# Cogito2012/OpenTAL

Hardware: AMD Instinct MI355X
Metric: clips/sec training step, 256-frame THUMOS14 clips (higher is better)
Workload: dtype bf16

## Files before the change

### opental_amd/csrc/conv1a_wgrad.inc

```
struct W1aArgs {
    ConvArgs c;
    int nblocks, bps;
};

template <bool DYH>
__global__ __launch_bounds__(256, 2) void conv1a_wgrad_direct_kernel(const W1aArgs d) {
    constexpr int PITCH = C1_PITCH;
    constexpr int PATCH = 2 * C1_NR * PITCH;
    constexpr int AP = 192 * 2 + 16;
    __shared__ __attribute__((aligned(16))) unsigned char lds[PATCH + 64 * AP];
    unsigned char* const patch = lds;
    unsigned char* const dyT = lds + PATCH;
    const ConvArgs& a = d.c;
    const ConvGeom& g = a.g;
    const int tid = threadIdx.x, lane = tid & 63;
    const int wave = __builtin_amdgcn_readfirstlane(tid >> 6);
    const TileId tile = xcd_tile(false);
    const int dt = tile.x, split = tile.y;
    const int blk_begin = split * d.bps, blk_end = min(d.nblocks, blk_begin + d.bps);
    const int tiles_h = g.Ho / 2, tiles_t = g.To / 2;
    const int HWo = g.Ho * g.Wo;
    const auto rx = __builtin_amdgcn_make_buffer_rsrc(const_cast<float*>(a.x), 0, (int)a.src_bytes, 0x00020000);
    const auto rdy = __builtin_amdgcn_make_buffer_rsrc(const_cast<float*>(a.dy), 0, (int)a.dy_bytes, 0x00020000);

    for (int i = tid; i < PATCH / 16; i += 256) reinterpret_cast<uint4*>(patch)[i] = make_uint4(0u, 0u, 0u, 0u);

    constexpr int X_ITEMS = 2 * C1_NR * 24, X_ITERS = (X_ITEMS + 255) / 256;
    int xrel[X_ITERS], xlds[X_ITERS], xpr[X_ITERS];
#pragma unroll
    for (int i = 0; i < X_ITERS; ++i) {
        const int item = tid + 256 * i;
        const int pl = item / (C1_NR * 24), rem = item - pl * (C1_NR * 24), rr = rem / 24, q = rem - rr * 24;
        xrel[i] = ((2 * pl) * g.Hi + rr) * g.Wi + 4 * q;
        xlds[i] = item < X_ITEMS ? (pl * C1_NR + rr) * PITCH + (4 * q + 2) * 8 : -1;
        xpr[i] = (pl << 8) | rr;
    }
    constexpr int A_ITERS = DYH ? 64 * 24 / 256 : 64 * 48 / 256;
    unsigned avo[A_ITERS];
    int alds[A_ITERS];
#pragma unroll
    for (int j = 0; j < A_ITERS; ++j) {
        const int item = tid + 256 * j;
        if constexpr (DYH) {
            const int co = item / 24, rem = item - co * 24, run = rem / 6, o = rem - run * 6;
            avo[j] = co < a.M ? (unsigned)(((int64_t)co * g.y_cs + (run >> 1) * HWo + (run & 1) * g.Wo + 8 * o) * 2) : 0xffffffffu;
            alds[j] = co * AP + (run * 48 + 8 * o) * 2;
        } else {
            const int co = item / 48, rem = item - co * 48, run = rem / 12, q = rem - run * 12;
            avo[j] = co < a.M ? (unsigned)(((int64_t)co * g.y_cs + (run >> 1) * HWo + (run & 1) * g.Wo + 4 * q) * 4) : 0xffffffffu;
            alds[j] = co * AP + (run * 48 + 4 * q) * 2;
        }
    }
    const int grp = wave & 1, khalf = wave >> 1;
    const int dh0 = 4 * grp;
    const int lanex = (2 * (8 * (lane >> 5) + ((lane & 15) >> 2)) + 4 * ((lane >> 4) & 1) + (lane & 3)) * 8;
    const unsigned char* const arow = dyT + (lane & 31) * AP + (lane >> 5) * 16;
    typedef __attribute__((address_space(3))) unsigned char lds_byte;
    lds_byte* const xl = (lds_byte*)patch + lanex + dh0 * PITCH;

    int xoffs[6], aoffs[6];
#pragma unroll
    for (int s2 = 0; s2 < 6; ++s2) {
        const int s = 2 * s2 + khalf;
        const int run = s / 3, w16 = s - run * 3, tl = run >> 1, hl = run & 1;
        xoffs[s2] = __builtin_amdgcn_readfirstlane((tl * C1_NR + 2 * hl) * PITCH + (2 * 16 * w16) * 8);
        aoffs[s2] = __builtin_amdgcn_readfirstlane(s * 32);
    }
    f32x16 acc[2][4];
#pragma unroll
    for (int i = 0; i < 2; ++i)
#pragma unroll
        for (int j = 0; j < 4; ++j)
#pragma unroll
            for (int r = 0; r < 16; ++r) acc[i][j][r] = 0.f;

    float4 xv[X_ITERS][3];
    Words4 ra[A_ITERS];
    auto load = [&](int blk) {
        int bid = blk;
        const int th = bid % tiles_h; bid /= tiles_h;
        const int tt0 = bid % tiles_t;
        const int b = bid / tiles_t;
        const int to0 = tt0 * 2, ho0 = th * 2;
        const int ti0 = 2 * to0 - g.pt + dt, hi0 = 2 * ho0 - g.ph;
        const int64_t xb0 = (int64_t)b * g.x_bs + ((int64_t)ti0 * g.Hi + hi0) * g.Wi;
#pragma unroll
        for (int i = 0; i < X_ITERS; ++i) {
            const int pl = xpr[i] >> 8, rr = xpr[i] & 255;
            const bool ok = xlds[i] >= 0 && (unsigned)(ti0 + 2 * pl) < (unsigned)g.Ti && (unsigned)(hi0 + rr) < (unsigned)g.Hi;
            const unsigned vo = ok ? (unsigned)((xb0 + xrel[i]) * 4) : 0xffffffffu;
#pragma unroll
            for (int ci = 0; ci < 3; ++ci) {
                const Words4 v = __builtin_bit_cast(Words4, __builtin_amdgcn_raw_buffer_load_b128(rx, vo, (int)(ci * g.x_cs * 4), 0));
                xv[i][ci] = make_float4(__uint_as_float(v.a), __uint_as_float(v.b), __uint_as_float(v.c), __uint_as_float(v.d));
            }
        }
        const int ybase = (int)(((int64_t)b * g.y_bs + (int64_t)to0 * HWo + ho0 * g.Wo) * (DYH ? 2 : 4));
#pragma unroll
        for (int j = 0; j < A_ITERS; ++j)
            ra[j] = __builtin_bit_cast(Words4, __builtin_amdgcn_raw_buffer_load_b128(rdy, avo[j], ybase, 0));
    };
    if (blk_begin < blk_end) load(blk_begin);
    for (int blk = blk_begin; blk < blk_end; ++blk) {
        __syncthreads();
#pragma unroll
        for (int i = 0; i < X_ITERS; ++i) {
            if (xlds[i] < 0) continue;
            uint2* dst = reinterpret_cast<uint2*>(patch + xlds[i]);
            dst[0] = make_uint2(cvt_pk_bf16(xv[i][0].x, xv[i][1].x), cvt_pk_bf16(xv[i][2].x, 0.f));
            dst[1] = make_uint2(cvt_pk_bf16(xv[i][0].y, xv[i][1].y), cvt_pk_bf16(xv[i][2].y, 0.f));
            dst[2] = make_uint2(cvt_pk_bf16(xv[i][0].z, xv[i][1].z), cvt_pk_bf16(xv[i][2].z, 0.f));
            dst[3] = make_uint2(cvt_pk_bf16(xv[i][0].w, xv[i][1].w), cvt_pk_bf16(xv[i][2].w, 0.f));
        }
#pragma unroll
        for (int j = 0; j < A_ITERS; ++j) {
            if constexpr (DYH) {
                *reinterpret_cast<Words4*>(dyT + alds[j]) = ra[j];
            } else {
                Words2 pk;
                pk.a = cvt_pk_bf16(__builtin_bit_cast(float, ra[j].a), __builtin_bit_cast(float, ra[j].b));
                pk.b = cvt_pk_bf16(__builtin_bit_cast(float, ra[j].c), __builtin_bit_cast(float, ra[j].d));
                *reinterpret_cast<Words2*>(dyT + alds[j]) = pk;
            }
        }
        __syncthreads();
        if (blk + 1 < blk_end) load(blk + 1);
#pragma unroll
        for (int s2 = 0; s2 < 6; ++s2) {
            const bf16x8 av0 = *reinterpret_cast<const bf16x8*>(arow + aoffs[s2]);
            const bf16x8 av1 = *reinterpret_cast<const bf16x8*>(arow + 32 * AP + aoffs[s2]);
#pragma unroll
            for (int j = 0; j < 4; ++j) {
                if (j == 3 && grp) continue;
                const v4s16 lo = __builtin_amdgcn_ds_read_tr16_b64_v4i16(
                    (__attribute__((address_space(3))) v4s16*)(xl + xoffs[s2] + j * PITCH));
                const v4s16 hi = __builtin_amdgcn_ds_read_tr16_b64_v4i16(
                    (__attribute__((address_space(3))) v4s16*)(xl + xoffs[s2] + j * PITCH + 64));
                const bf16x8 bv = {lo[0], lo[1], lo[2], lo[3], hi[0], hi[1], hi[2], hi[3]};
                acc[0][j] = __builtin_amdgcn_mfma_f32_32x32x16_bf16(av0, bv, acc[0][j], 0, 0, 0);
                acc[1][j] = __builtin_amdgcn_mfma_f32_32x32x16_bf16(av1, bv, acc[1][j], 0, 0, 0);
            }
        }
    }

    float* const xch = reinterpret_cast<float*>(lds);
#pragma unroll
    for (int mt = 0; mt < 2; ++mt) {
        __syncthreads();
        if (khalf) {
#pragma unroll
            for (int j = 0; j < 4; ++j)
#pragma unroll
                for (int r = 0; r < 16; ++r) xch[((grp * 4 + j) * 16 + r) * 64 + lane] = acc[mt][j][r];
        }
        __syncthreads();
        if (!khalf) {
#pragma unroll
            for (int j = 0; j < 4; ++j)
#pragma unroll
                for (int r = 0; r < 16; ++r) acc[mt][j][r] += xch[((grp * 4 + j) * 16 + r) * 64 + lane];
        }
    }
    if (khalf) return;

    const bool slabs = a.splits > 1;
    const auto ro = __builtin_amdgcn_make_buffer_rsrc(slabs ? a.slab : a.out, 0, (int)(slabs ? a.slab_bytes : a.out_bytes), 0x00020000);
    const bool accum = !slabs && (a.flags & EPI_ACCUM);
    const int nn = lane & 31, dw = nn >> 2, ci = nn & 3;
#pragma unroll
    for (int j = 0; j < 4; ++j) {
        if (j == 3 && grp) continue;
        const int dh = dh0 + j;
        const unsigned col = (unsigned)(ci * 343 + dt * 49 + dh * 7 + dw);
        const bool okn = ci < 3 && dw < 7;
#pragma unroll
        for (int mt = 0; mt < 2; ++mt)
#pragma unroll
            for (int r = 0; r < 16; ++r) {
                const int m = mt * 32 + (r & 3) + 8 * (r >> 2) + 4 * (lane >> 5);
                const unsigned vo = (okn && m < a.M) ? (((unsigned)(slabs ? split : 0) * (unsigned)a.M + (unsigned)m) * (unsigned)a.N + col) * 4u : 0xffffffffu;
                float v = acc[mt][j][r];
                if (accum) v += __uint_as_float(__builtin_amdgcn_raw_buffer_load_b32(ro, vo, 0, 0));
                __builtin_amdgcn_raw_buffer_store_b32(__float_as_uint(v), ro, vo, 0, 0);
            }
    }
}

int launch_conv1a_wgrad(ConvArgs& a, void* ws, size_t ws_bytes, hipStream_t st) {
    const ConvGeom& g = a.g;
    W1aArgs d;
    d.nblocks = g.B * (g.To / 2) * (g.Ho / 2);
    int splits = OTAL_OPT("OTAL_W1A_SPLITS") > 0 ? OTAL_OPT("OTAL_W1A_SPLITS") : 73;
    if (splits > d.nblocks) splits = d.nblocks;
    const size_t slab1 = (size_t)a.M * a.N * sizeof(float);
    if (splits > 1 && (!ws || ws_bytes < (size_t)splits * slab1)) {
        splits = ws ? (int)(ws_bytes / slab1) : 1;
        if (splits < 2) splits = 1;
    }
    d.bps = (d.nblocks + splits - 1) / splits;
    splits = (d.nblocks + d.bps - 1) / d.bps;
    a.splits = splits;
    a.k_per_split = d.bps;
    a.slab = splits > 1 ? (float*)ws : nullptr;
    a.src_bytes = (unsigned)gather_extent_bytes(g, MODE_FWD);
    a.dy_bytes = (unsigned)(gather_extent_bytes(g, MODE_DGRAD) >> (a.half ? 1 : 0));
    a.flags &= ~EPI_NPAD8;
    set_epilogue_extents<MODE_WGRAD>(a);
    if ((splits > 1 ? a.slab_bytes : a.out_bytes) == 0u) return OTAL_E_UNSUPPORTED;
    d.c = a;
    if (a.half) hipLaunchKernelGGL(conv1a_wgrad_direct_kernel<true>, dim3(7, splits), dim3(256), 0, st, d);
    else hipLaunchKernelGGL(conv1a_wgrad_direct_kernel<false>, dim3(7, splits), dim3(256), 0, st, d);
    if (int e = otal_launch_status()) return e;
    if (splits > 1) return launch_splitk_reduce<MODE_WGRAD>(a, st);
    return 0;
}
```

### opental_amd/csrc/conv_select.h

```cpp
#pragma once
#include <stddef.h>
#include <stdint.h>
#include "conv_index.h"
#include "options.h"

namespace {

enum { MODE_FWD = 0, MODE_DGRAD = 1, MODE_WGRAD = 2 };

constexpr int C1_TT = 2, C1_TR = 2, C1_WO = 48;
constexpr int C1T_TT = 4, C1T_TR = 4;
constexpr int W1_TC = 128;
constexpr int PJ_HW = 36;
constexpr int PW_KS = 32;
constexpr size_t TAB_PAD = 64;
constexpr int CHUNK_PAD = 16;
constexpr int PTAB_PAD = 64;

static inline size_t align256(size_t v) { return (v + 255) & ~(size_t)255; }
static inline size_t tab_bytes(int K) { return (((size_t)K + TAB_PAD) * (2 * sizeof(int)) + 255) & ~(size_t)255; }
static inline int chunk_kp(int K) { return (K + 31) / 32 * 32; }
static inline size_t chunk_tab_bytes(int K) { return align256(((size_t)chunk_kp(K) / 8 + CHUNK_PAD) * (2 * sizeof(int))); }
static inline size_t chunk_wp_bytes(int M, int BM, int K) {
    return align256(((size_t)((M + BM - 1) / BM * BM) * chunk_kp(K) + 64) * sizeof(unsigned short));
}
static inline size_t ptab_bytes(const ConvGeom& g, int cw) {
    return align256(((size_t)g.B * conv_out_positions(g) / cw + PTAB_PAD) * (2 * sizeof(int)));
}
static inline int64_t gather_extent_bytes(const ConvGeom& g, int mode, int esz = 4) {
    if (mode == MODE_FWD) return esz * ((int64_t)(g.B - 1) * g.x_bs + (int64_t)(g.Cin - 1) * g.x_cs + conv_in_positions(g));
    return esz * ((int64_t)(g.B - 1) * g.y_bs + (int64_t)(g.Cout - 1) * g.y_cs + conv_out_positions(g));
}

static inline int choose_bm(int M, bool tall = false) {
    if (tall && M % 192 == 0) return 192;
    const int cand[4] = {128, 96, 64, 32};
    const double pen[4] = {1.00, 1.03, 1.10, 1.30};
    int best = 128;
    double bc = 1e30;
    for (int i = 0; i < 4; ++i) {
        const double c = (double)((M + cand[i] - 1) / cand[i] * cand[i]) * pen[i];
        if (c < bc) { bc = c; best = cand[i]; }
    }
    return best;
}

static inline int choose_splits(int tiles, int K, int prec = 1, bool wgrad = false) {
    const bool wv = wgrad && prec;
    const int target = wv ? 2048 : 512;
    const int minsteps = wv ? 16 : (prec ? 8 : 4);
    const int cap = wv ? 1024 : 384;
    if (tiles >= target * 3 / 4) return 1;
    int want = (target + tiles - 1) / tiles;
    int maxs = K / (minsteps * 32);
    if (maxs < 1) maxs = 1;
    int s = want < maxs ? want : maxs;
    return s < 1 ? 1 : (s > cap ? cap : s);
}

static inline bool conv1a_half_out_ok(const ConvGeom& g, const void* y) {
    return g.y_bs % 8 == 0 && g.y_cs % 8 == 0 && (reinterpret_cast<uintptr_t>(y) & 15) == 0;
}
static inline bool conv1a_direct_eligible(const ConvGeom& g, int mode, int prec, const void* x) {
    if (!prec || mode != MODE_FWD || g.nlev > 1 || OTAL_OPT("OTAL_CONV_NO1A")) return false;
    if (g.Cin != 3 || g.kt != 7 || g.kh != 7 || g.kw != 7 || g.st != 2 || g.sh != 2 || g.sw != 2) return false;
    if (g.pt != 2 || g.ph != 2 || g.pw != 2 || g.Wi != 96 || g.Wo != C1_WO || g.Hi != 2 * g.Ho || g.Ti != 2 * g.To) return false;
    if (g.To % C1_TT || g.Ho % C1_TR || g.x_bs % 4 || g.x_cs % 4 || (reinterpret_cast<uintptr_t>(x) & 15)) return false;
    return (int64_t)g.B * g.To * g.Ho * g.Wo < (1LL << 31);
}
static inline int conv1a_tile_eligible(int To, int Ho) {
    return To % C1T_TT == 0 && Ho % C1T_TR == 0 && !OTAL_OPT("OTAL_CONV_1A_NOTILE");
}
static inline bool conv1a_wgrad_eligible(const ConvGeom& g, int prec, const void* x, const void* dy) {
    if (!prec || g.nlev > 1 || OTAL_OPT("OTAL_CONV_NO1AW")) return false;
    if (g.Cin != 3 || g.Cout > 64 || g.kt != 7 || g.kh != 7 || g.kw != 7 || g.st != 2 || g.sh != 2 || g.sw != 2) return false;
    if (g.pt != 2 || g.ph != 2 || g.pw != 2 || g.Wi != 96 || g.Wo != C1_WO || g.Hi != 2 * g.Ho || g.Ti != 2 * g.To) return false;
    if (g.To % 2 || g.Ho % 2 || g.x_bs % 4 || g.x_cs % 4 || g.y_bs % 4 || g.y_cs % 4) return false;
    if ((reinterpret_cast<uintptr_t>(x) & 15) || (reinterpret_cast<uintptr_t>(dy) & 15)) return false;
    const int64_t ex = gather_extent_bytes(g, MODE_FWD), ey = gather_extent_bytes(g, MODE_DGRAD);
    return ex > 0 && ey > 0 && ex < (1LL << 31) && ey < (1LL << 31);
}

static inline bool proj_fwd_eligible(const ConvGeom& g, int mode, int prec, const void* x, const void* w) {
    if (!prec || mode != MODE_FWD || g.nlev > 1 || OTAL_OPT("OTAL_CONV_NOPROJ")) return false;
    if (g.kt != 1 || g.st != 1 || g.kh != g.Hi || g.kw != g.Wi || g.Ho != 1 || g.Wo != 1 || g.To != g.Ti) return false;
    if (g.Hi * g.Wi != PJ_HW || g.ph != 0 || g.pw != 0 || g.pt != 0 || g.Cin % 4) return false;
    if (((uintptr_t)x & 3) || ((uintptr_t)w & 3)) return false;
    const int64_t ex = gather_extent_bytes(g, MODE_FWD), ew = 4 * (int64_t)g.Cout * g.Cin * PJ_HW;
    return ex > 0 && ex < (1LL << 31) && ew < (1LL << 31);
}
static inline bool proj_wgrad_eligible(const ConvGeom& g, int prec, const void* x, const void* dy) {
    if (!prec || g.nlev > 1 || OTAL_OPT("OTAL_CONV_NOPROJW")) return false;
    if (g.kt != 1 || g.st != 1 || g.kh != g.Hi || g.kw != g.Wi || g.Ho != 1 || g.Wo != 1 || g.To != g.Ti) return false;
    if (g.ph != 0 || g.pw != 0 || g.pt != 0 || g.Hi * g.Wi < 2) return false;
    if (g.To % PW_KS || g.y_cs < g.To || (g.y_cs & 3) || (g.y_bs & 3)) return false;
    if (((uintptr_t)x & 15) || ((uintptr_t)dy & 15) || (g.x_bs & 3) || (g.x_cs & 3)) return false;
    const int64_t ex = gather_extent_bytes(g, MODE_FWD), ey = gather_extent_bytes(g, MODE_DGRAD);
    const int64_t eo = 4 * (int64_t)g.Cout * g.Cin * g.Hi * g.Wi;
    return ex > 0 && ey > 0 && ex < (1LL << 31) && ey < (1LL << 31) && eo < (1LL << 31);
}

static inline bool conv1d_tile_eligible(const ConvGeom& g, int mode, int prec, const void* src, bool emask) {
    if (!prec || mode == MODE_WGRAD || OTAL_OPT("OTAL_CONV_NO1DTILE")) return false;
    if (g.Hi != 1 || g.Wi != 1 || g.Ho != 1 || g.Wo != 1 || g.kh != 1 || g.kw != 1 || g.st != 1 || g.To != g.Ti) return false;
    if (!((g.kt == 1 && g.pt == 0) || (g.kt == 3 && g.pt == 1))) return false;
    if (g.Ti > 4096) return false;
    if ((mode == MODE_FWD ? g.Cout : g.Cin) > 2048) return false;
    const int C = mode == MODE_FWD ? g.Cin : g.Cout;
    if (C % 128) return false;
    if (mode == MODE_DGRAD && emask) return false;
    if (((uintptr_t)src & 3)) return false;
    const int64_t ext = gather_extent_bytes(g, mode);
    return ext > 0 && ext < (1LL << 31);
}
static inline int wgrad1d_chunks(const ConvGeom& g) { return (g.Ti + W1_TC - 1) / W1_TC; }
static inline bool wgrad1d_eligible(const ConvGeom& g, int prec, const void* x, const void* dy) {
    if (!prec || OTAL_OPT("OTAL_CONV_NOW1D")) return false;
    if (g.Hi != 1 || g.Wi != 1 || g.Ho != 1 || g.Wo != 1 || g.kh != 1 || g.kw != 1 || g.st != 1 || g.To != g.Ti) return false;
    if (!((g.kt == 1 && g.pt == 0) || (g.kt == 3 && g.pt == 1))) return false;
    if (g.Cin % 64 || (g.x_bs | g.x_cs | g.y_bs | g.y_cs) & 1) return false;
    if ((reinterpret_cast<uintptr_t>(x) | reinterpret_cast<uintptr_t>(dy)) & 7) return false;
    return (int64_t)g.B * wgrad1d_chunks(g) <= 1024;
}

static inline bool chunk_eligible(const ConvGeom& g, int mode, int prec) {
    if (!prec || mode == MODE_WGRAD) return false;
    const int C = mode == MODE_FWD ? g.Cin : g.Cout;
    if (C % 8 && !(mode == MODE_FWD && g.kw >= 3)) return false;
    const int64_t ext = gather_extent_bytes(g, mode);
    return ext > 0 && ext < (int64_t)0xfffffff0u;
}
static inline bool conv1x1_stream_eligible(const ConvGeom& g, int mode) {
    if (OTAL_OPT("OTAL_CONV_NO1X1STREAM")) return false;
    if (g.kt != 1 || g.kh != 1 || g.kw != 1 || g.st != 1 || g.sh != 1 || g.sw != 1 || g.nlev > 1) return false;
    const int64_t P = conv_out_positions(g);
    if (P != conv_in_positions(g) || P % 128) return false;
    const int C = mode == MODE_FWD ? g.Cin : g.Cout;
    return C % 8 == 0;
}

static inline int direct_bm(const ConvGeom& g, int M) {
    if (M % 96 == 0) return 96;
    if (M > 96) {
        const int64_t nt = (int64_t)g.B * conv_out_positions(g) / 256;
        const int64_t w64 = (M + 63) / 64 * nt, w96 = (M + 95) / 96 * nt;
        if (w64 <= 512 && (w96 + 255) / 256 * 96 < (w64 + 255) / 256 * 64) return 96;
    }
    if (M % 64 == 0) return 64;
    if (M <= 32) return 32;
    const int pad64 = (M + 63) / 64 * 64;
    return (pad64 - M) * 100 <= M * 34 ? 64 : 0;
}
static inline int direct_bnp(const ConvGeom& g, int M) {
    const int BM = direct_bm(g, M);
    if (!BM) return 0;
    const int64_t tm = (M + BM - 1) / BM, NP = (int64_t)g.B * conv_out_positions(g);
    const int min_tiles = OTAL_OPT("OTAL_CONV_DIRECT_MINTILES");
    if (BM == 96 && conv_out_positions(g) % 512 == 0 && tm * (NP / 512) >= OTAL_OPT("OTAL_CONV_DIRECT_MINTILES512")) return 512;
    if (tm * (NP / 256) >= min_tiles) return 256;
    if (tm * (NP / 128) >= min_tiles) return 128;
    return 0;
}
static inline bool direct_eligible(const ConvGeom& g, int mode, int prec, int M) {
    if (OTAL_OPT("OTAL_CONV_NODIRECT") || !prec || mode == MODE_WGRAD || g.nlev > 1) return false;
    if (g.kt != 3 || g.kh != 3 || g.kw != 3 || g.st != 1 || g.sh != 1 || g.sw != 1 || g.pt != 1 || g.ph != 1 || g.pw != 1) return false;
    if (g.To != g.Ti || g.Ho != g.Hi || g.Wo != g.Wi || g.Wi > 24) return false;
    const int P = conv_out_positions(g);
    const int C = mode == MODE_FWD ? g.Cin : g.Cout;
    if (P % 256 || C % 16 || !direct_bnp(g, M)) return false;
    const int64_t ext = gather_extent_bytes(g, mode);
    return ext > 0 && ext < (1LL << 31);
}
static inline size_t direct_wp_bytes(const ConvGeom& g, int M, int C) {
    const int BM = direct_bm(g, M);
    return align256((size_t)((M + BM - 1) / BM * BM) * C * 27 * 2 + 1024);
}

static inline bool wgrad_direct_eligible(const ConvGeom& g, int prec, const void* x, const void* dy) {
    if (!prec || OTAL_OPT("OTAL_CONV_NOWDIRECT") || g.nlev > 1) return false;
    if (g.kt != 3 || g.kh != 3 || g.kw != 3 || g.st != 1 || g.sh != 1 || g.sw != 1 || g.pt != 1 || g.ph != 1 || g.pw != 1) return false;
    if (g.To != g.Ti || g.Ho != g.Hi || g.Wo != g.Wi) return false;
    const bool planes6 = g.Wi == 6 && g.Hi == 6 && g.Ti % 4 == 0;
    const bool planes3 = g.Wi == 3 && g.Hi == 3 && g.Ti % 16 == 0;
    if (!((g.Wi == 24 && g.Hi % 4 == 0) || (g.Wi == 12 && g.Hi == 12) || planes6 || planes3) || g.Cin % 2) return false;
    if (g.Cin < (planes3 ? 32 : 64) || g.Cout < 64) return false;
    if (((uintptr_t)x & 15) || ((uintptr_t)dy & 15) || g.x_cs % 4 || g.x_bs % 4 || g.y_cs % 4 || g.y_bs % 4) return false;
    const int64_t ex = gather_extent_bytes(g, MODE_FWD), ey = gather_extent_bytes(g, MODE_DGRAD);
    return ex > 0 && ey > 0 && ex < (1LL << 31) && ey < (1LL << 31);
}
static inline bool wgrad1x1_wide_eligible(const ConvGeom& g, int prec, const void* x, const void* dy) {
    if (!prec || g.nlev > 1 || OTAL_OPT("OTAL_CONV_NOW1X1")) return false;
    if (g.kt != 1 || g.kh != 1 || g.kw != 1 || g.st != 1 || g.sh != 1 || g.sw != 1) return false;
    if (g.To != g.Ti || g.Ho != g.Hi || g.Wo != g.Wi) return false;
    if (g.Hi == 1 && g.Wi == 1) return false;
    if (conv_out_positions(g) % 32 || (int64_t)g.Cout * g.Cin > (1 << 20)) return false;
    if (((uintptr_t)x & 3) || ((uintptr_t)dy & 3)) return false;
    const int64_t ex = gather_extent_bytes(g, MODE_FWD), ey = gather_extent_bytes(g, MODE_DGRAD);
    return ex > 0 && ey > 0 && ex < (1LL << 31) && ey < (1LL << 31);
}
static inline bool wgrad_pair_mode(const ConvGeom& g, int prec) {
    if (!prec || g.nlev > 1) return false;
    if (g.sw != 2 || g.st > 2 || g.sh > 2 || g.kw > 7 || g.pw > 3 || g.Wo % 8 || conv_out_positions(g) % 32) return false;
    if (g.Wi - (2 * (g.Wo - 8) - g.pw + 6) < 12) return false;
    const int64_t ex = 4 * ((int64_t)(g.B - 1) * g.x_bs + (int64_t)(g.Cin - 1) * g.x_cs + conv_in_positions(g));
    const int64_t ey = 4 * ((int64_t)(g.B - 1) * g.y_bs + (int64_t)(g.Cout - 1) * g.y_cs + conv_out_positions(g));
    return ex > 0 && ey > 0 && ex < (int64_t)0xffffff00u && ey < (int64_t)0xfffffff0u;
}
static inline int wgrad_vector_width(const ConvGeom& g, int prec) {
    if (!prec) return 0;
    if (g.st != 1 || g.sh != 1 || g.sw != 1 || g.nlev > 1) return 0;
    if (g.To != g.Ti || g.Ho != g.Hi || g.Wo != g.Wi) return 0;
    if ((g.kw != 1 && g.kw != 3) || g.pw != (g.kw - 1) / 2) return 0;
    if (conv_out_positions(g) % 32) return 0;
    const int64_t ex = 4 * ((int64_t)(g.B - 1) * g.x_bs + (int64_t)(g.Cin - 1) * g.x_cs + conv_in_positions(g));
    const int64_t ey = 4 * ((int64_t)(g.B - 1) * g.y_bs + (int64_t)(g.Cout - 1) * g.y_cs + conv_out_positions(g));
    if (ex <= 0 || ey <= 0 || ex >= (int64_t)0xfffffff0u || ey >= (int64_t)0xfffffff0u) return 0;
    if (g.kt == 1 && g.kh == 1 && g.kw == 1) return 8;
    if (g.Wi % 8 == 0) return 8;
    if (g.Wi % 4 == 0) return 4;
    if (g.Wi % 2 == 0) return 2;
    return 0;
}

enum ConvKernel {
    CK_GENERIC,
    CK_PROJ, CK_CONV1A, CK_CONV1D_TILE, CK_DIRECT, CK_CHUNKED,
    CK_CONV1A_WGRAD, CK_PROJ_WGRAD, CK_WGRAD_DIRECT, CK_WGRAD1X1, CK_WGRAD_VECTOR, CK_WGRAD1D,
};
static inline const char* conv_kernel_name(int kernel) {
    switch (kernel) {
        case CK_GENERIC: return "generic";
        case CK_PROJ: return "proj";
        case CK_CONV1A: return "conv1a";
        case CK_CONV1D_TILE: return "conv1d_tile";
        case CK_DIRECT: return "direct";
        case CK_CHUNKED: return "chunked";
        case CK_CONV1A_WGRAD: return "conv1a_wgrad";
        case CK_PROJ_WGRAD: return "proj_wgrad";
        case CK_WGRAD_DIRECT: return "wgrad_direct";
        case CK_WGRAD1X1: return "wgrad1x1_wide";
        case CK_WGRAD_VECTOR: return "vector";
        case CK_WGRAD1D: return "wgrad1d";
    }
    return "?";
}
enum ConvPrologue { PRO_NONE = 0, PRO_CHUNK = 1, PRO_PTAB = 2, PRO_DIRECT = 3 };

struct ConvQuery {
    ConvGeom g;
    int mode;
    int precision;
    int accumulate;
    int has_mask;
    uintptr_t x, w, dy, out, mask;
};
struct ConvStep {
    int kernel;
    int cw;
    bool next;
};
struct ConvPlan {
    int n;
    ConvStep step[8];
    int prologue;
};

static inline int conv_step_prologue(int kernel) {
    switch (kernel) {
        case CK_CONV1D_TILE: case CK_CHUNKED: return PRO_CHUNK;
        case CK_DIRECT: return PRO_DIRECT;
        case CK_WGRAD_VECTOR: return PRO_PTAB;
        default: return PRO_NONE;
    }
}

static inline int conv_prologue_layout(const ConvGeom& g, int mode, int prec) {
    if (mode == MODE_WGRAD) return wgrad_pair_mode(g, prec) || wgrad_vector_width(g, prec) ? PRO_PTAB : PRO_NONE;
    if (proj_fwd_eligible(g, mode, prec, nullptr, nullptr)) return PRO_NONE;
    if (conv1a_direct_eligible(g, mode, prec, nullptr)) return PRO_NONE;
    if (direct_eligible(g, mode, prec, mode == MODE_FWD ? g.Cout : g.Cin)) return PRO_DIRECT;
    return chunk_eligible(g, mode, prec) ? PRO_CHUNK : PRO_NONE;
}
static inline size_t conv_prologue_bytes(const ConvGeom& g, int mode, int prec) {
    const int layout = conv_prologue_layout(g, mode, prec);
    const int M = mode == MODE_FWD ? g.Cout : g.Cin;
    if (layout == PRO_CHUNK) {
        const bool kwv = mode == MODE_FWD && (g.Cin % 8) != 0;
        const int K = mode == MODE_FWD ? (kwv ? g.Cin * g.kt * g.kh * 8 : g.Cin * conv_kvol(g)) : g.Cout * conv_kvol(g);
        return chunk_tab_bytes(K) + chunk_wp_bytes(M, choose_bm(M, !kwv), K);
    }
    if (layout == PRO_PTAB) return ptab_bytes(g, g.sw == 2 ? 8 : wgrad_vector_width(g, prec));
    if (layout == PRO_DIRECT) return direct_wp_bytes(g, M, mode == MODE_FWD ? g.Cin : g.Cout);
    return 0;
}

static inline void conv_plan_half(const ConvQuery& q, ConvPlan& p) {
    const ConvGeom& g = q.g;
    const void* px = (const void*)(q.mode == MODE_DGRAD ? q.out : q.x);
    const void* py = (const void*)(q.mode == MODE_FWD ? q.out : q.dy);
    auto add = [&p](int kernel, bool next, int cw = 0) { p.step[p.n++] = ConvStep{kernel, cw, next}; };
    if (!(q.precision & 1) || !(q.precision & 4) || q.accumulate) return;
    if (((uintptr_t)px | (uintptr_t)py) & 15) return;
    if (q.mode == MODE_DGRAD && q.has_mask && (!(q.precision & 16) || (q.mask & 15))) return;
    if (g.nlev > 1) return;
    if (conv_out_positions(g) % 8 || conv_in_positions(g) % 8 || g.x_bs % 8 || g.x_cs % 8 || g.y_bs % 8 || g.y_cs % 8) return;
    if (q.mode == MODE_FWD || q.mode == MODE_DGRAD) {
        const int M = q.mode == MODE_FWD ? g.Cout : g.Cin, C = q.mode == MODE_FWD ? g.Cin : g.Cout;
        if (direct_eligible(g, q.mode, 1, M) && !(g.Wi & 1)) add(CK_DIRECT, false);
        else if (chunk_eligible(g, q.mode, 1) && C % 8 == 0 && conv_in_positions(g) == conv_out_positions(g)) add(CK_CHUNKED, false);
        return;
    }
    const int cw = wgrad_vector_width(g, 1);
    if (wgrad_direct_eligible(g, 1, px, py)) add(CK_WGRAD_DIRECT, true);
    else if (wgrad1x1_wide_eligible(g, 1, px, py)) add(CK_WGRAD1X1, true);
    if (cw) add(CK_WGRAD_VECTOR, false, cw);
}

static inline ConvPlan conv_plan(const ConvQuery& q) {
    ConvPlan p = {};
    const ConvGeom& g = q.g;
    const int prec = q.precision & 1, half = (q.precision >> 2) & 1;
    p.prologue = conv_prologue_layout(g, q.mode, prec);
    if (q.precision & 8) { conv_plan_half(q, p); return p; }
    const void *x = (const void*)q.x, *w = (const void*)q.w, *dy = (const void*)q.dy, *out = (const void*)q.out;
    auto add = [&p](int kernel, bool next, int cw = 0) { p.step[p.n++] = ConvStep{kernel, cw, next}; };
    if (q.mode == MODE_WGRAD) {
        if (conv1a_wgrad_eligible(g, prec, x, dy) && (!half || g.y_bs % 8 + g.y_cs % 8 == 0)) add(CK_CONV1A_WGRAD, !half);
        if (half) return p;
        if (proj_wgrad_eligible(g, prec, x, dy)) add(CK_PROJ_WGRAD, true);
        if (wgrad_direct_eligible(g, prec, x, dy)) add(CK_WGRAD_DIRECT, true);
        if (wgrad1x1_wide_eligible(g, prec, x, dy)) add(CK_WGRAD1X1, true);
        if (wgrad_pair_mode(g, prec)) { add(CK_WGRAD_VECTOR, false, 8); return p; }
        if (const int cw = wgrad_vector_width(g, prec)) { add(CK_WGRAD_VECTOR, false, cw); return p; }
        if (wgrad1d_eligible(g, prec, x, dy)) add(CK_WGRAD1D, true);
        add(CK_GENERIC, false);
        return p;
    }
    const int M = q.mode == MODE_FWD ? g.Cout : g.Cin;
    if (q.mode == MODE_FWD) {
        if (proj_fwd_eligible(g, q.mode, prec, x, w)) add(CK_PROJ, true);
        if (half) {
            if (conv1a_direct_eligible(g, q.mode, prec, x) && conv1a_half_out_ok(g, out)) add(CK_CONV1A, false);
            else if (direct_eligible(g, q.mode, prec, M) && conv1a_half_out_ok(g, out)) add(CK_DIRECT, false);
            return p;
        }
        if (conv1a_direct_eligible(g, q.mode, prec, x)) { add(CK_CONV1A, false); return p; }
    }
    if (half) return p;
    if (conv1d_tile_eligible(g, q.mode, prec, q.mode == MODE_FWD ? x : dy, q.has_mask)) add(CK_CONV1D_TILE, true);
    if (direct_eligible(g, q.mode, prec, M)) add(CK_DIRECT, false);
    else if (chunk_eligible(g, q.mode, prec)) add(CK_CHUNKED, false);
    else add(CK_GENERIC, false);
    return p;
}

static inline int conv_half_storage(const ConvGeom& g, int mode, int precision) {
    if (!(precision & 1) || g.y_bs % 8 || g.y_cs % 8) return 0;
    ConvQuery q = {};
    q.g = g;
    q.mode = mode;
    q.precision = precision | 4;
    const ConvPlan p = conv_plan(q);
    for (int i = 0; i < p.n; ++i)
        if (p.step[i].kernel != CK_PROJ) return 1;
    return 0;
}

}
```

### opental_amd/csrc/options.h

```cpp
#pragma once

struct OtalOption { const char* name; int dflt; };
constexpr OtalOption OTAL_OPTIONS[] = {
    {"OTAL_CONV_1A_NOTILE", 0},           {"OTAL_CONV_1A_WGS", 0},
    {"OTAL_CONV_DIRECT_MINTILES", 140},   {"OTAL_CONV_DIRECT_MINTILES512", 512},
    {"OTAL_CONV_DIRECT_XPF2", 3},         {"OTAL_CONV_NO1A", 0},
    {"OTAL_CONV_NO1AW", 0},               {"OTAL_CONV_NO1DTILE", 0},
    {"OTAL_CONV_NO1X1STREAM", 0},         {"OTAL_CONV_NODIRECT", 0},
    {"OTAL_CONV_NOPROJ", 0},              {"OTAL_CONV_NOPROJW", 0},
    {"OTAL_CONV_NOW1D", 0},               {"OTAL_CONV_NOW1X1", 0},
    {"OTAL_CONV_NOWDIRECT", 0},           {"OTAL_LOSS_NOSTAGE", 0},
    {"OTAL_POOL_NO133", 0},               {"OTAL_POOL_NOROWS", 0},
    {"OTAL_W1A_SPLITS", 0},               {"OTAL_WDIRECT_BLOCKS", 0},
};
constexpr int OTAL_NUM_OPTIONS = sizeof(OTAL_OPTIONS) / sizeof(OTAL_OPTIONS[0]);
constexpr bool otal_streq(const char* a, const char* b) { return *a == *b && (*a == 0 || otal_streq(a + 1, b + 1)); }
constexpr int otal_option_index(const char* name, int i = 0) {
    return i == OTAL_NUM_OPTIONS ? -1 : otal_streq(OTAL_OPTIONS[i].name, name) ? i : otal_option_index(name, i + 1);
}
int* otal_option_slot(int index);
#define OTAL_OPT(name) ([]() -> int {                                                                              \
    constexpr int index_ = otal_option_index(name);                                                              \
    static_assert(index_ >= 0, "unknown option " name " (options.h: OTAL_OPTIONS)");                               \
    static int* const slot_ = otal_option_slot(index_);                                                          \
    return *slot_;                                                                                               \
}())
```

Baseline: 1011.

## Add 4x4-block conv1a weight-gradient kernel with pipelined dy ring and LDS patch reuse

```diff
diff --git a/opental_amd/csrc/conv1a_wgrad.inc b/opental_amd/csrc/conv1a_wgrad.inc
--- a/opental_amd/csrc/conv1a_wgrad.inc
+++ b/opental_amd/csrc/conv1a_wgrad.inc
@@ -186,10 +186,13 @@
     }
 }
 
+#include "conv1a_wgrad_blocks.inc"
+
 int launch_conv1a_wgrad(ConvArgs& a, void* ws, size_t ws_bytes, hipStream_t st) {
     const ConvGeom& g = a.g;
     W1aArgs d;
-    d.nblocks = g.B * (g.To / 2) * (g.Ho / 2);
+    const bool blocks4 = conv1a_wgrad_blocks_eligible(g.To, g.Ho);
+    d.nblocks = blocks4 ? g.B * (g.To / 4) * (g.Ho / 4) : g.B * (g.To / 2) * (g.Ho / 2);
     int splits = OTAL_OPT("OTAL_W1A_SPLITS") > 0 ? OTAL_OPT("OTAL_W1A_SPLITS") : 73;
     if (splits > d.nblocks) splits = d.nblocks;
     const size_t slab1 = (size_t)a.M * a.N * sizeof(float);
@@ -208,7 +211,10 @@
     set_epilogue_extents<MODE_WGRAD>(a);
     if ((splits > 1 ? a.slab_bytes : a.out_bytes) == 0u) return OTAL_E_UNSUPPORTED;
     d.c = a;
-    if (a.half) hipLaunchKernelGGL(conv1a_wgrad_direct_kernel<true>, dim3(7, splits), dim3(256), 0, st, d);
+    if (blocks4) {
+        if (a.half) hipLaunchKernelGGL(conv1a_wgrad_blocks_kernel<true>, dim3(7, splits), dim3(256), 0, st, d);
+        else hipLaunchKernelGGL(conv1a_wgrad_blocks_kernel<false>, dim3(7, splits), dim3(256), 0, st, d);
+    } else if (a.half) hipLaunchKernelGGL(conv1a_wgrad_direct_kernel<true>, dim3(7, splits), dim3(256), 0, st, d);
     else hipLaunchKernelGGL(conv1a_wgrad_direct_kernel<false>, dim3(7, splits), dim3(256), 0, st, d);
     if (int e = otal_launch_status()) return e;
     if (splits > 1) return launch_splitk_reduce<MODE_WGRAD>(a, st);
diff --git a/opental_amd/csrc/conv1a_wgrad_blocks.inc b/opental_amd/csrc/conv1a_wgrad_blocks.inc
--- /dev/null
+++ b/opental_amd/csrc/conv1a_wgrad_blocks.inc
@@ -0,0 +1,212 @@
+constexpr int W1B_NPL = 4, W1B_NR = 13;
+
+template <bool DYH>
+__global__ __launch_bounds__(256, 2) void conv1a_wgrad_blocks_kernel(const W1aArgs d) {
+    constexpr int PITCH = C1_PITCH;
+    constexpr int PLANE = W1B_NR * PITCH;
+    constexpr int HALF = 2 * PLANE;
+    constexpr int PATCH = W1B_NPL * PLANE;
+    constexpr int ESZ = DYH ? 2 : 4;
+    constexpr int G = DYH ? 4 : 2;
+    constexpr int NA = DYH ? 1 : 2;
+    constexpr int STEPS = 12;
+    constexpr int NG = 2 * STEPS / G;
+    constexpr int NS = 3;
+    static_assert(STEPS % G == 0 && 4 % G == 0 && NG % NS == 0, "the ring's slots are compile-time indices");
+    __shared__ __attribute__((aligned(16))) unsigned char lds[PATCH];
+    const ConvArgs& a = d.c;
+    const ConvGeom& g = a.g;
+    const int tid = threadIdx.x, lane = tid & 63;
+    const int wave = __builtin_amdgcn_readfirstlane(tid >> 6);
+    const TileId tile = xcd_tile(false);
+    const int dt = tile.x, split = tile.y;
+    const int blk_begin = split * d.bps, blk_end = min(d.nblocks, blk_begin + d.bps);
+    const int tiles_h = g.Ho / 4, tiles_t = g.To / 4;
+    const int HWo = g.Ho * g.Wo;
+    const auto rx = __builtin_amdgcn_make_buffer_rsrc(const_cast<float*>(a.x), 0, (int)a.src_bytes, 0x00020000);
+    const auto rdy = __builtin_amdgcn_make_buffer_rsrc(const_cast<float*>(a.dy), 0, (int)a.dy_bytes, 0x00020000);
+
+    for (int i = tid; i < PATCH / 16; i += 256) reinterpret_cast<uint4*>(lds)[i] = make_uint4(0u, 0u, 0u, 0u);
+    __syncthreads();
+
+    constexpr int X_ITEMS = 2 * W1B_NR * 24, X_ITERS = (X_ITEMS + 255) / 256;
+    int xitem[X_ITERS];
+#pragma unroll
+    for (int i = 0; i < X_ITERS; ++i) {
+        const int item = tid + 256 * i;
+        const int pl = item / (W1B_NR * 24), rem = item - pl * (W1B_NR * 24), rr = rem / 24, q = rem - rr * 24;
+        xitem[i] = item < X_ITEMS ? (pl | rr << 4 | q << 8) : -1;
+    }
+    const int mt = wave & 1, khalf = wave >> 1;
+    const int lanex = (2 * (8 * (lane >> 5) + ((lane & 15) >> 2)) + 4 * ((lane >> 4) & 1) + (lane & 3)) * 8;
+    typedef __attribute__((address_space(3))) unsigned char lds_byte;
+    lds_byte* const xl = (lds_byte*)lds + lanex + khalf * PLANE;
+    const int co = mt * 32 + (lane & 31);
+    const unsigned avo = co < a.M ? (unsigned)(((int64_t)co * g.y_cs + 8 * (lane >> 5)) * ESZ) : 0xffffffffu;
+
+    f32x16 acc[7];
+#pragma unroll
+    for (int j = 0; j < 7; ++j)
+#pragma unroll
+        for (int r = 0; r < 16; ++r) acc[j][r] = 0.f;
+
+    auto decode = [&](int blk, int& b, int& tt0, int& th) {
+        int bid = blk;
+        th = bid % tiles_h; bid /= tiles_h;
+        tt0 = bid % tiles_t;
+        b = bid / tiles_t;
+    };
+    auto ybase_of = [&](int blk) {
+        int b, tt0, th;
+        decode(blk, b, tt0, th);
+        return (int)(((int64_t)b * g.y_bs + (int64_t)(4 * tt0 + khalf) * HWo + 4 * th * g.Wo) * ESZ);
+    };
+    const int yhalf = 2 * HWo * ESZ;
+    float4 xs[2][3];
+    Words4 ra[NS][G * NA];
+    auto load_xi = [&](int set, int blk, int p, int i) {
+        int b, tt0, th;
+        decode(blk, b, tt0, th);
+        const int ti0 = 2 * (4 * tt0 + 2 * p) - g.pt + dt, hi0 = 2 * (4 * th) - g.ph;
+        const int64_t xb0 = (int64_t)b * g.x_bs + ((int64_t)ti0 * g.Hi + hi0) * g.Wi;
+        int it = xitem[i];
+        asm volatile("" : "+v"(it));
+        const int pl = it & 15, rr = (it >> 4) & 15, q = (it >> 8) & 31;
+        const bool ok = it >= 0 && (unsigned)(ti0 + 2 * pl) < (unsigned)g.Ti && (unsigned)(hi0 + rr) < (unsigned)g.Hi;
+        const unsigned vo = ok ? (unsigned)((xb0 + ((2 * pl) * g.Hi + rr) * g.Wi + 4 * q) * 4) : 0xffffffffu;
+#pragma unroll
+        for (int ci = 0; ci < 3; ++ci) {
+            const Words4 v = __builtin_bit_cast(Words4, __builtin_amdgcn_raw_buffer_load_b128(rx, vo, (int)(ci * g.x_cs * 4), 0));
+            xs[set][ci] = make_float4(__uint_as_float(v.a), __uint_as_float(v.b), __uint_as_float(v.c), __uint_as_float(v.d));
+        }
+    };
+    auto store_xi = [&](int set, int p, int i) {
+        int it = xitem[i];
+        asm volatile("" : "+v"(it));
+        if (it < 0) return;
+        uint2* dst = reinterpret_cast<uint2*>(lds + p * HALF + (it & 15) * PLANE + ((it >> 4) & 15) * PITCH + ((it >> 8) & 31) * 32 + 16);
+        const float4 c0 = xs[set][0], c1 = xs[set][1], c2 = xs[set][2];
+        dst[0] = make_uint2(cvt_pk_bf16(c0.x, c1.x), cvt_pk_bf16(c2.x, 0.f));
+        dst[1] = make_uint2(cvt_pk_bf16(c0.y, c1.y), cvt_pk_bf16(c2.y, 0.f));
+        dst[2] = make_uint2(cvt_pk_bf16(c0.z, c1.z), cvt_pk_bf16(c2.z, 0.f));
+        dst[3] = make_uint2(cvt_pk_bf16(c0.w, c1.w), cvt_pk_bf16(c2.w, 0.f));
+    };
+    auto load_granule = [&](int gi, int yb) {
+        const int j0 = gi * G;
+        const int so = yb + (j0 / STEPS) * yhalf + 16 * (j0 % STEPS) * ESZ;
+#pragma unroll
+        for (int i = 0; i < G * NA; ++i)
+            ra[gi % NS][i] = __builtin_bit_cast(Words4, __builtin_amdgcn_raw_buffer_load_b128(rdy, avo, so + (i / NA) * 16 * ESZ + (i % NA) * 16, 0));
+    };
+    auto frag_a = [&](int j) {
+        const int slot = (j / G) % NS, i = j % G;
+        if constexpr (DYH) {
+            return __builtin_bit_cast(bf16x8, ra[slot][i]);
+        } else {
+            const Words4 lo = ra[slot][2 * i], hi = ra[slot][2 * i + 1];
+            Words4 pk;
+            pk.a = cvt_pk_bf16(__builtin_bit_cast(float, lo.a), __builtin_bit_cast(float, lo.b));
+            pk.b = cvt_pk_bf16(__builtin_bit_cast(float, lo.c), __builtin_bit_cast(float, lo.d));
+            pk.c = cvt_pk_bf16(__builtin_bit_cast(float, hi.a), __builtin_bit_cast(float, hi.b));
+            pk.d = cvt_pk_bf16(__builtin_bit_cast(float, hi.c), __builtin_bit_cast(float, hi.d));
+            return __builtin_bit_cast(bf16x8, pk);
+        }
+    };
+
+    bf16x8 bv[7];
+    int yb_cur = 0;
+    if (blk_begin < blk_end) {
+        yb_cur = ybase_of(blk_begin);
+#pragma unroll
+        for (int gi = 0; gi < NS; ++gi) load_granule(gi, yb_cur);
+        load_xi(0, blk_begin, 0, 0);
+        load_xi(1, blk_begin, 0, 1);
+        store_xi(0, 0, 0);
+        load_xi(0, blk_begin, 0, 2);
+        store_xi(1, 0, 1);
+        store_xi(0, 0, 2);
+        load_xi(0, blk_begin, 1, 0);
+        load_xi(1, blk_begin, 1, 1);
+    }
+    for (int blk = blk_begin; blk < blk_end; ++blk) {
+        const bool more = blk + 1 < blk_end;
+        const int yb_next = more ? ybase_of(blk + 1) : yb_cur;
+#pragma unroll
+        for (int q = 0; q < 6; ++q) {
+            const int p = q / 3;
+            lds_byte* const xh = xl + p * HALF;
+            auto read_b = [&](int jj, int r) {
+                const int xoff = (2 * (jj / 3) + r) * PITCH + (2 * 16 * (jj % 3)) * 8;
+                const v4s16 lo = __builtin_amdgcn_ds_read_tr16_b64_v4i16((__attribute__((address_space(3))) v4s16*)(xh + xoff));
+                const v4s16 hi = __builtin_amdgcn_ds_read_tr16_b64_v4i16((__attribute__((address_space(3))) v4s16*)(xh + xoff + 64));
+                return bf16x8{lo[0], lo[1], lo[2], lo[3], hi[0], hi[1], hi[2], hi[3]};
+            };
+            if (q % 3 == 0) __syncthreads();
+            if (q < 3) store_xi(q & 1, 1, q);
+            else if (more) store_xi(q & 1, 0, q - 3);
+            if (q == 0) load_xi(q & 1, blk, 1, 2);
+            else if (more) {
+                if (q < 4) load_xi(q & 1, blk + 1, 0, q - 1);
+                else load_xi(q & 1, blk + 1, 1, q - 4);
+            }
+            if (q % 3 == 0) {
+#pragma unroll
+                for (int r = 0; r < 7; ++r) bv[r] = read_b(0, r);
+            }
+#pragma unroll
+            for (int s4 = 0; s4 < 4; ++s4) {
+                const int jj = (q % 3) * 4 + s4, j = p * STEPS + jj;
+                const bf16x8 av = frag_a(j);
+                if (j % G == G - 1) {
+                    const int gi = j / G + NS;
+                    if (gi < NG) load_granule(gi, yb_cur);
+                    else load_granule(gi - NG, yb_next);
+                }
+#pragma unroll
+                for (int r = 0; r < 7; ++r) {
+                    acc[r] = __builtin_amdgcn_mfma_f32_32x32x16_bf16(av, bv[r], acc[r], 0, 0, 0);
+                    if (jj + 1 < STEPS) bv[r] = read_b(jj + 1, r);
+                }
+            }
+        }
+        yb_cur = yb_next;
+    }
+
+    float* const xch = reinterpret_cast<float*>(lds);
+#pragma unroll
+    for (int t = 0; t < 2; ++t) {
+        __syncthreads();
+        if (khalf && mt == t) {
+#pragma unroll
+            for (int j = 0; j < 7; ++j)
+#pragma unroll
+                for (int r = 0; r < 16; ++r) xch[(j * 16 + r) * 64 + lane] = acc[j][r];
+        }
+        __syncthreads();
+        if (!khalf && mt == t) {
+#pragma unroll
+            for (int j = 0; j < 7; ++j)
+#pragma unroll
+                for (int r = 0; r < 16; ++r) acc[j][r] += xch[(j * 16 + r) * 64 + lane];
+        }
+    }
+    if (khalf) return;
+
+    const bool slabs = a.splits > 1;
+    const auto ro = __builtin_amdgcn_make_buffer_rsrc(slabs ? a.slab : a.out, 0, (int)(slabs ? a.slab_bytes : a.out_bytes), 0x00020000);
+    const bool accum = !slabs && (a.flags & EPI_ACCUM);
+    const int nn = lane & 31, dw = nn >> 2, ci = nn & 3;
+    const bool okn = ci < 3 && dw < 7;
+#pragma unroll
+    for (int dh = 0; dh < 7; ++dh) {
+        const unsigned col = (unsigned)(ci * 343 + dt * 49 + dh * 7 + dw);
+#pragma unroll
+        for (int r = 0; r < 16; ++r) {
+            const int m = mt * 32 + (r & 3) + 8 * (r >> 2) + 4 * (lane >> 5);
+            const unsigned vo = (okn && m < a.M) ? (((unsigned)(slabs ? split : 0) * (unsigned)a.M + (unsigned)m) * (unsigned)a.N + col) * 4u : 0xffffffffu;
+            float v = acc[dh][r];
+            if (accum) v += __uint_as_float(__builtin_amdgcn_raw_buffer_load_b32(ro, vo, 0, 0));
+            __builtin_amdgcn_raw_buffer_store_b32(__float_as_uint(v), ro, vo, 0, 0);
+        }
+    }
+}
diff --git a/opental_amd/csrc/conv_select.h b/opental_amd/csrc/conv_select.h
--- a/opental_amd/csrc/conv_select.h
+++ b/opental_amd/csrc/conv_select.h
@@ -10,6 +10,7 @@
 
 constexpr int C1_TT = 2, C1_TR = 2, C1_WO = 48;
 constexpr int C1T_TT = 4, C1T_TR = 4;
+constexpr int C1W_TT = 4, C1W_TR = 4;
 constexpr int W1_TC = 128;
 constexpr int PJ_HW = 36;
 constexpr int PW_KS = 32;
@@ -79,6 +80,10 @@
     if ((reinterpret_cast<uintptr_t>(x) & 15) || (reinterpret_cast<uintptr_t>(dy) & 15)) return false;
     const int64_t ex = gather_extent_bytes(g, MODE_FWD), ey = gather_extent_bytes(g, MODE_DGRAD);
     return ex > 0 && ey > 0 && ex < (1LL << 31) && ey < (1LL << 31);
+}
+
+static inline int conv1a_wgrad_blocks_eligible(int To, int Ho) {
+    return To % C1W_TT == 0 && Ho % C1W_TR == 0 && !OTAL_OPT("OTAL_CONV_1AW_NOBLOCKS");
 }
 
 static inline bool proj_fwd_eligible(const ConvGeom& g, int mode, int prec, const void* x, const void* w) {
diff --git a/opental_amd/csrc/options.h b/opental_amd/csrc/options.h
--- a/opental_amd/csrc/options.h
+++ b/opental_amd/csrc/options.h
@@ -2,6 +2,7 @@
 
 struct OtalOption { const char* name; int dflt; };
 constexpr OtalOption OTAL_OPTIONS[] = {
+    {"OTAL_CONV_1AW_NOBLOCKS", 0},
     {"OTAL_CONV_1A_NOTILE", 0},           {"OTAL_CONV_1A_WGS", 0},
     {"OTAL_CONV_DIRECT_MINTILES", 140},   {"OTAL_CONV_DIRECT_MINTILES512", 512},
     {"OTAL_CONV_DIRECT_XPF2", 3},         {"OTAL_CONV_NO1A", 0},
```

Result: no change. 1015 (median of 3 runs) (+0.4%).
